# paroj/aruco

Measured on AMD Instinct MI355X. Metric: frames/sec at 1920×1080, higher is better.
Workload: dtype u8; 1 GPU; 1920x1080 synthetic stream, ~20 markers/frame, threshold+contour+decode+LINES, no pose (config 2); distinct_frames_per_gpu=1024, markers_rendered_per_frame=20, batches_in_flight=5, build=src=0ab799cac5660a2f flags=[], gpu_max_hw_queues=4, parallelism=frames sharded 1 stream/GPU

## Files before the change

### aruco_amd/csrc/decode_device.h

```cpp
#pragma once
#include "internal.h"

namespace ah {

__device__ inline bool solve8(double* A, double* b) {
    const int n = 8;
    for (int c = 0; c < n; c++) {
        int piv = c;
        double best = fabs(A[c * n + c]);
        for (int r = c + 1; r < n; r++) {
            double v = fabs(A[r * n + c]);
            if (v > best) best = v, piv = r;
        }
        if (best == 0) return false;
        if (piv != c) {
            for (int k = 0; k < n; k++) {
                double t = A[c * n + k];
                A[c * n + k] = A[piv * n + k];
                A[piv * n + k] = t;
            }
            double t = b[c];
            b[c] = b[piv];
            b[piv] = t;
        }
        double inv = 1.0 / A[c * n + c];
        for (int r = c + 1; r < n; r++) {
            double f = A[r * n + c] * inv;
            if (f == 0) continue;
            for (int k = c; k < n; k++) A[r * n + k] -= f * A[c * n + k];
            b[r] -= f * b[c];
        }
    }
    for (int r = n - 1; r >= 0; r--) {
        double s = b[r];
        for (int k = r + 1; k < n; k++) s -= A[r * n + k] * b[k];
        b[r] = s / A[r * n + r];
    }
    return true;
}

__device__ inline void perspective_transform_solve(const float* src, const float* dst, double* A, double* b, bool float_products = false) {
    for (int i = 0; i < 64; i++) A[i] = 0;
    for (int i = 0; i < 4; i++) {
        const float sx = src[2 * i], sy = src[2 * i + 1], dx = dst[2 * i], dy = dst[2 * i + 1];
        double* r0 = A + i * 8;
        double* r1 = A + (i + 4) * 8;
        r0[0] = r1[3] = sx;
        r0[1] = r1[4] = sy;
        r0[2] = r1[5] = 1;
        if (float_products) {
            r0[6] = -sx * dx;
            r0[7] = -sy * dx;
            r1[6] = -sx * dy;
            r1[7] = -sy * dy;
        } else {
            r0[6] = -(double)sx * dx;
            r0[7] = -(double)sy * dx;
            r1[6] = -(double)sx * dy;
            r1[7] = -(double)sy * dy;
        }
        b[i] = dx;
        b[i + 4] = dy;
    }
    if (!solve8(A, b))
        for (int i = 0; i < 8; i++) b[i] = 0;
}

constexpr int HOMOGRAPHY_GROUP = 16;
template <int G>
struct LaneMatT {
    double* base;
    int lane;
    __device__ __forceinline__ double& operator[](int k) const { return base[k * G + (lane & (G - 1))]; }
};
using LaneMat = LaneMatT<HOMOGRAPHY_GROUP>;
template <int G>
constexpr int homography_lds_doubles() { return 64 * G + 8 * G; }
constexpr int HOMOGRAPHY_LDS_DOUBLES = homography_lds_doubles<HOMOGRAPHY_GROUP>();

template <typename Mat>
__device__ __forceinline__ void homography_lane(const int16_t* qx, const int16_t* qy, int ws, const Mat& A, const Mat& b, double* iM) {
    const double d = (double)(float)(ws - 1);
    const double dxs[4] = {0, d, d, 0}, dys[4] = {0, 0, d, d};
    for (int i = 0; i < 64; i++) A[i] = 0;
    for (int i = 0; i < 4; i++) {
        const double sx = (double)(float)qx[i], sy = (double)(float)qy[i], dx = dxs[i], dy = dys[i];
        const int r0 = i * 8, r1 = (i + 4) * 8;
        A[r0 + 0] = sx, A[r1 + 3] = sx;
        A[r0 + 1] = sy, A[r1 + 4] = sy;
        A[r0 + 2] = 1, A[r1 + 5] = 1;
        A[r0 + 6] = -sx * dx;
        A[r0 + 7] = -sy * dx;
        A[r1 + 6] = -sx * dy;
        A[r1 + 7] = -sy * dy;
        b[i] = dx;
        b[i + 4] = dy;
    }
    bool ok = true;
    for (int c = 0; c < 8 && ok; c++) {
        int piv = c;
        double best = fabs(A[c * 8 + c]);
        for (int r = c + 1; r < 8; r++) {
            double v = fabs(A[r * 8 + c]);
            if (v > best) best = v, piv = r;
        }
        if (best == 0) {
            ok = false;
            break;
        }
        if (piv != c) {
            for (int k = 0; k < 8; k++) {
                double t = A[c * 8 + k];
                A[c * 8 + k] = A[piv * 8 + k];
                A[piv * 8 + k] = t;
            }
            double t = b[c];
            b[c] = b[piv];
            b[piv] = t;
        }
        const double inv = 1.0 / A[c * 8 + c];
        for (int r = c + 1; r < 8; r++) {
            const double f = A[r * 8 + c] * inv;
            if (f == 0) continue;
            for (int k = c; k < 8; k++) A[r * 8 + k] -= f * A[c * 8 + k];
            b[r] -= f * b[c];
        }
    }
    double m[9];
    if (ok) {
        for (int r = 7; r >= 0; r--) {
            double sacc = b[r];
            for (int k = r + 1; k < 8; k++) sacc -= A[r * 8 + k] * b[k];
            b[r] = sacc / A[r * 8 + r];
        }
        for (int i = 0; i < 8; i++) m[i] = b[i];
    } else {
        for (int i = 0; i < 8; i++) m[i] = 0;
    }
    m[8] = 1.0;
    double det = m[0] * (m[4] * m[8] - m[5] * m[7]) - m[1] * (m[3] * m[8] - m[5] * m[6]) + m[2] * (m[3] * m[7] - m[4] * m[6]);
    det = det != 0 ? 1. / det : 0;
    iM[0] = (m[4] * m[8] - m[5] * m[7]) * det;
    iM[1] = (m[2] * m[7] - m[1] * m[8]) * det;
    iM[2] = (m[1] * m[5] - m[2] * m[4]) * det;
    iM[3] = (m[5] * m[6] - m[3] * m[8]) * det;
    iM[4] = (m[0] * m[8] - m[2] * m[6]) * det;
    iM[5] = (m[2] * m[3] - m[0] * m[5]) * det;
    iM[6] = (m[3] * m[7] - m[4] * m[6]) * det;
    iM[7] = (m[1] * m[6] - m[0] * m[7]) * det;
    iM[8] = (m[0] * m[4] - m[1] * m[3]) * det;
}

__device__ __forceinline__ int hamm_rows(const uint32_t v[5]) {
    const uint32_t words[4] = {0x01, 0x1D, 0x12, 0x0E};
    int dist = 0;
#pragma unroll
    for (int y = 0; y < 5; y++) {
        int best = 100000;
#pragma unroll
        for (int p = 0; p < 4; p++) best = min(best, __popc(v[y] ^ words[p]));
        dist += best;
    }
    return dist;
}

__device__ __forceinline__ void fiducial_decode_word(unsigned long long m, int* id_out, int* nrot_out) {
    int id = -1, nrot = 0;
    unsigned long long border = 0x7Full | (0x7Full << 42);
#pragma unroll
    for (int y = 1; y < 6; y++) border |= (1ull << (7 * y)) | (1ull << (7 * y + 6));
    if ((m & border) == 0) {
        uint32_t cur[5], best[5];
#pragma unroll
        for (int y = 0; y < 5; y++) cur[y] = (uint32_t)(m >> (7 * (y + 1) + 1)) & 31u, best[y] = cur[y];
        int min_dist = hamm_rows(cur);
#pragma unroll
        for (int r = 1; r < 4; r++) {
            uint32_t nxt[5];
#pragma unroll
            for (int i = 0; i < 5; i++) {
                nxt[i] = 0;
#pragma unroll
                for (int j = 0; j < 5; j++) nxt[i] |= ((cur[4 - j] >> i) & 1u) << j;
            }
#pragma unroll
            for (int i = 0; i < 5; i++) cur[i] = nxt[i];
            const int dd = hamm_rows(cur);
            if (dd < min_dist) {
                min_dist = dd, nrot = r;
#pragma unroll
                for (int i = 0; i < 5; i++) best[i] = cur[i];
            }
        }
        if (min_dist == 0) {
            id = 0;
#pragma unroll
            for (int y = 0; y < 5; y++) id |= (int)((((best[y] >> 1) & 1u) << 1) | ((best[y] >> 3) & 1u)) << (2 * (4 - y));
        }
    }
    *id_out = id, *nrot_out = nrot;
}

constexpr int CELLS_PITCH = 8;
constexpr int cell_vote_rank(int sw) { return (sw * sw) / 2 + 1; }

__device__ __forceinline__ void cells_decode_wave(const uint8_t* patch, int ws, int thr, int lane, int* id_out, int* nrot_out) {
    const int sw = ws / 7;
    const int half = cell_vote_rank(sw) - 1;
    bool white = false;
    if (lane < 49) {
        const int cy = lane / 7, cx = lane - cy * 7;
        int cnt = 0;
        if (sw == 8 && (((size_t)patch | (size_t)ws) & 7) == 0) {
#pragma unroll
            for (int y = 0; y < 8; y++) {
                const uint2 w = *(const uint2*)(patch + (cy * 8 + y) * ws + cx * 8);
#pragma unroll
                for (int b = 0; b < 4; b++) cnt += (int)((w.x >> (8 * b)) & 0xFFu) > thr, cnt += (int)((w.y >> (8 * b)) & 0xFFu) > thr;
            }
        } else {
            for (int y = 0; y < sw; y++)
                for (int x = 0; x < sw; x++) cnt += patch[(cy * sw + y) * ws + cx * sw + x] > thr;
        }
        white = cnt > half;
    }
    const unsigned long long m = __ballot(white);
    int id = -1, nrot = 0;
    if (lane == 0) fiducial_decode_word(m, &id, &nrot);
    *id_out = id, *nrot_out = nrot;
}

}
```

### aruco_amd/csrc/k_contours.hip

```cpp
#include <algorithm>

#include "bits_tiles.h"
#include "internal.h"
#include "decode_device.h"

namespace ah {

__device__ __forceinline__ int first_dir(uint32_t m, int s_end) {
    int s = s_end;
    do {
        s = (s - 1) & 7;
        if ((m >> s) & 1) break;
    } while (s != s_end);
    return s == s_end ? -1 : s;
}

__device__ __forceinline__ bool run_rule_tiles(const uint64_t* __restrict__ tiles, int tnx, int x, int y, int hole) {
    int avail, avail_up;
    const uint64_t mid = tb_row64(tiles, tnx, x, y, &avail), up = tb_row64(tiles, tnx, x, y - 1, &avail_up);
    if (!hole) {
        int L = (~mid) ? __builtin_ctzll(~mid) : 64;
        L = min(L, avail);
        const int hi = min(L, avail - 1);
        const uint64_t m = hi >= 2 ? ((hi >= 63 ? ~0ull : ((1ull << (hi + 1)) - 1ull)) & ~3ull) : 0ull;
        return (up & m) == 0;
    }
    int L = mid ? __builtin_ctzll(mid) : 64;
    L = min(L, avail);
    const int hi = min(L - 1, avail - 1);
    const uint64_t m = hi >= 1 ? ((hi >= 63 ? ~0ull : ((1ull << (hi + 1)) - 1ull)) & ~1ull) : 0ull;
    return (~up & m) == 0;
}

struct CandArgs {
    const uint64_t* tiles;
    int tnx, tny;
    int width, height;
    uint32_t* trig_cnt;
    uint2* raw;
    uint32_t* raw_cnt;
    uint32_t* counters;
    uint32_t cap_raw;
    int grid_mask;
    uint32_t* hash;
    uint32_t hash_size;
};

constexpr int CAND_THREADS = 256;
constexpr int CAND_STAGE = 512;

__global__ __launch_bounds__(CAND_THREADS) void candidates_kernel(CandArgs a) {
    throughput_bound_priority();
    __shared__ uint2 s_keep[CAND_STAGE];
    __shared__ uint32_t s_n, s_base;
    const int plane = blockIdx.y;
    const uint64_t* __restrict__ tiles = a.tiles + (size_t)plane * a.tnx * a.tny;
    const int ntx = a.tnx - 1, nty = a.tny - 1;
    const int ntiles = ntx * nty;
    const uint64_t COL0 = 0x0101010101010101ull, COL7 = 0x8080808080808080ull;
    for (uint32_t i = blockIdx.x * CAND_THREADS + threadIdx.x; i < a.hash_size; i += gridDim.x * CAND_THREADS) a.hash[(size_t)plane * a.hash_size + i] = 0xFFFFFFFFu;
    uint2* const out = a.raw + (size_t)plane * a.cap_raw;
    uint32_t* const out_cnt = a.raw_cnt + plane * TRIG_CNT_STRIDE;

    auto stage = [&](uint2 rec) {
        const uint32_t ls = atomicAdd(&s_n, 1u);
        if (ls < CAND_STAGE) {
            s_keep[ls] = rec;
        } else {
            const uint32_t slot = atomicAdd(out_cnt, 1u);
            if (slot < a.cap_raw)
                out[slot] = rec;
            else
                flag_overflow(a.counters, a.trig_cnt, plane, ST_TRIG_OVERFLOW);
        }
    };

    for (int i0 = blockIdx.x * CAND_THREADS; i0 < ntiles; i0 += gridDim.x * CAND_THREADS) {
        if (threadIdx.x == 0) s_n = 0;
        __syncthreads();
        const int i = i0 + threadIdx.x;
        if (i < ntiles) {
            const int ty = i / ntx, tx = i - ty * ntx;
            const uint64_t* t = tiles + (size_t)ty * a.tnx + tx;
            const uint64_t T = t[0];
            const uint64_t L = tx > 0 ? t[-1] : 0ull;
            const uint64_t U = ty > 0 ? t[-a.tnx] : 0ull, UL = (ty > 0 && tx > 0) ? t[-a.tnx - 1] : 0ull, UR = ty > 0 ? t[-a.tnx + 1] : 0ull;
            const uint64_t Rt = t[1];
            if (T | L | U) {
                const uint64_t Wn = ((T << 1) & ~COL0) | ((L >> 7) & COL0);
                const uint64_t N = (T << 8) | (U >> 56), NLt = (L << 8) | (UL >> 56), NRt = (Rt << 8) | (UR >> 56);
                const uint64_t NW = ((N << 1) & ~COL0) | ((NLt >> 7) & COL0);
                const uint64_t NE = ((N >> 1) & ~COL7) | ((NRt << 7) & COL7);
                const int jmax = a.width - 2 - 8 * tx, imax = a.height - 2 - 8 * ty;
                const uint64_t colm = (jmax >= 7 ? 0xFFull : ((1ull << (jmax + 1)) - 1ull)) * COL0;
                const uint64_t rowm = imax >= 7 ? ~0ull : ((1ull << (8 * (imax + 1))) - 1ull);
                const uint64_t outer = T & ~(Wn | NW | N | NE);
                const uint64_t hole = ~T & Wn & N & colm & rowm;
                const uint32_t base = ((uint32_t)(8 * ty) << 16) | (uint32_t)(8 * tx);
                uint64_t rsel = 0, csel = 0;
#pragma unroll
                for (int q = 0; q < 8; q++) {
                    if (((8 * ty + q) & a.grid_mask) == 0) rsel |= 0xFFull << (8 * q);
                    if (((8 * tx + q) & a.grid_mask) == 0) csel |= COL0 << q;
                }
                const uint64_t crW = T & ~Wn & (rsel | outer);
                const uint64_t crE = ~T & Wn & (rsel | hole);
                const uint64_t crN = T & ~N & csel;
                const uint64_t crS = N & ~T & csel;
                for (int kind = 0; kind < 4; kind++) {
                    uint64_t m = kind == 0 ? crW : kind == 1 ? crE : kind == 2 ? crN : crS;
                    while (m) {
                        const int b = __builtin_ctzll(m);
                        m &= m - 1;
                        const uint32_t z = base + ((uint32_t)(b >> 3) << 16) + (uint32_t)(b & 7);
                        uint32_t pos, code, cand = 0;
                        if (kind == 0) pos = z, code = 2u, cand = (uint32_t)(outer >> b) & 1u;
                        else if (kind == 1) pos = z - 1u, code = 0u, cand = (uint32_t)(hole >> b) & 1u;
                        else if (kind == 2) pos = z, code = 1u;
                        else pos = z - 65536u, code = 3u;
                        stage(make_uint2(cand, (pos << 2) | code));
                    }
                }
            }
        }
        __syncthreads();
        if (threadIdx.x == 0 && s_n) s_base = atomicAdd(out_cnt, min(s_n, (uint32_t)CAND_STAGE));
        __syncthreads();
        const uint32_t n = min(s_n, (uint32_t)CAND_STAGE);
        for (uint32_t j = threadIdx.x; j < n; j += CAND_THREADS) {
            const uint32_t slot = s_base + j;
            if (slot < a.cap_raw)
                out[slot] = s_keep[j];
            else
                flag_overflow(a.counters, a.trig_cnt, plane, ST_TRIG_OVERFLOW);
        }
        __syncthreads();
    }
}

constexpr int CQ_CAP = 192;
constexpr int CS_CAP = 256;

struct SparseArgs {
    const uint64_t* tiles;
    const uint64_t* tile_bits;
    int tnx, tny, nstrips;
    int width, height;
    uint2* trig;
    uint32_t* trig_cnt;
    uint32_t* counters;
    uint32_t cap_trig;
    int drop_single;
};

__global__ __launch_bounds__(64) void candidates_sparse_kernel(SparseArgs a) {
    throughput_bound_priority();
    __shared__ uint32_t s_q[CQ_CAP];
    __shared__ uint2 s_keep[2][CS_CAP];
    __shared__ uint32_t s_n[2];
    const int plane = blockIdx.y, lane = threadIdx.x;
    const uint64_t* __restrict__ tiles = a.tiles + (size_t)plane * a.tnx * a.tny;
    const uint64_t* __restrict__ bits = a.tile_bits + (size_t)plane * a.tny * (2 * a.nstrips);
    const int ntx = a.tnx - 1, nty = a.tny - 1;
    const uint32_t half = a.cap_trig / 2;
    uint2* const out = a.trig + (size_t)plane * a.cap_trig;
    uint32_t* const out_cnt = a.trig_cnt + plane * TRIG_CNT_STRIDE;
    const uint64_t COL0 = 0x0101010101010101ull, COL7 = 0x8080808080808080ull;
    if (lane < 2) s_n[lane] = 0;
    __syncthreads();

    auto flush = [&]() {
        __syncthreads();
        for (int kind = 0; kind < 2; kind++) {
            const uint32_t n = min(s_n[kind], (uint32_t)CS_CAP);
            if (n == 0) continue;
            uint32_t base = 0;
            if (lane == 0) base = atomicAdd(&out_cnt[kind], n);
            base = (uint32_t)__builtin_amdgcn_readfirstlane((int)base);
            for (uint32_t j = lane; j < n; j += WAVE) {
                if (base + j < half)
                    out[(size_t)kind * half + base + j] = s_keep[kind][j];
                else
                    flag_overflow(a.counters, a.trig_cnt, plane, ST_TRIG_OVERFLOW);
            }
        }
        __syncthreads();
        if (lane < 2) s_n[lane] = 0;
        __syncthreads();
    };
    auto stage = [&](int kind, uint2 rec) {
        const uint32_t ls = atomicAdd(&s_n[kind], 1u);
        if (ls < CS_CAP) {
            s_keep[kind][ls] = rec;
        } else {
            const uint32_t slot = atomicAdd(&out_cnt[kind], 1u);
            if (slot < half)
                out[(size_t)kind * half + slot] = rec;
            else
                flag_overflow(a.counters, a.trig_cnt, plane, ST_TRIG_OVERFLOW);
        }
    };
    struct TileSet {
        uint64_t T, L, U, UL, UR, Rt;
        int tx, ty;
    };
    auto fetch = [&](bool live, uint32_t id) -> TileSet {
        TileSet q;
        q.ty = (int)(id >> 16), q.tx = (int)(id & 0xFFFFu);
        q.T = q.L = q.U = q.UL = q.UR = q.Rt = 0ull;
        if (live) {
            const uint64_t* t = tiles + (size_t)q.ty * a.tnx + q.tx;
            q.T = t[0];
            q.L = q.tx > 0 ? t[-1] : 0ull;
            q.U = q.ty > 0 ? t[-a.tnx] : 0ull, q.UL = (q.ty > 0 && q.tx > 0) ? t[-a.tnx - 1] : 0ull, q.UR = q.ty > 0 ? t[-a.tnx + 1] : 0ull;
            q.Rt = t[1];
        }
        return q;
    };
    auto evaluate = [&](bool live, const TileSet& q) {
        if (live) {
            const int ty = q.ty, tx = q.tx;
            const uint64_t T = q.T, L = q.L, U = q.U, UL = q.UL, UR = q.UR, Rt = q.Rt;
            const uint64_t Wn = ((T << 1) & ~COL0) | ((L >> 7) & COL0);
            const uint64_t N = (T << 8) | (U >> 56), NLt = (L << 8) | (UL >> 56), NRt = (Rt << 8) | (UR >> 56);
            const uint64_t NW = ((N << 1) & ~COL0) | ((NLt >> 7) & COL0);
            const uint64_t NE = ((N >> 1) & ~COL7) | ((NRt << 7) & COL7);
            const int jmax = a.width - 2 - 8 * tx, imax = a.height - 2 - 8 * ty;
            const uint64_t colm = (jmax >= 7 ? 0xFFull : (jmax < 0 ? 0ull : ((1ull << (jmax + 1)) - 1ull))) * COL0;
            const uint64_t rowm = imax >= 7 ? ~0ull : (imax < 0 ? 0ull : ((1ull << (8 * (imax + 1))) - 1ull));
            uint64_t outer = T & ~(Wn | NW | N | NE);
            const uint64_t hole = ~T & Wn & N & colm & rowm;
            if (a.drop_single) {
                const uint64_t E = ((T >> 1) & ~COL7) | ((Rt << 7) & COL7);
                const uint64_t lower = (T >> 8) | (Wn >> 8) | (E >> 8);
                outer &= ~(~(E | lower) & 0x00FFFFFFFFFFFFFFull);
            }
            const uint32_t base = ((uint32_t)(8 * ty) << 16) | (uint32_t)(8 * tx);
            uint64_t m = outer | hole;
            while (m) {
                const int b = __builtin_ctzll(m);
                m &= m - 1;
                const int qr = b >> 3, j = b & 7;
                const uint32_t kind = (uint32_t)(hole >> b) & 1u;
                const uint32_t mid = ((((uint32_t)(T >> (8 * qr)) & 0xFFu) | (((uint32_t)(Rt >> (8 * qr)) & 0xFFu) << 8)) >> j);
                const uint32_t up = ((((uint32_t)(N >> (8 * qr)) & 0xFFu) | (((uint32_t)(NRt >> (8 * qr)) & 0xFFu) << 8)) >> j);
                const int avail = 16 - j;
                const uint32_t pos = base + ((uint32_t)qr << 16) + (uint32_t)j;
                const uint32_t runbits = (kind ? mid : ~mid) | (1u << avail);
                const int Lr = __builtin_ctz(runbits);
                const int hi = kind ? min(Lr - 1, avail - 1) : min(Lr, avail - 1);
                const uint32_t span = ((2u << hi) - 1u) & (kind ? ~1u : ~3u);
                if (((kind ? ~up : up) & span) != 0) continue;
                if (Lr < avail || run_rule_tiles(tiles, a.tnx, (int)(pos & 0xFFFFu), (int)(pos >> 16), (int)kind)) stage((int)kind, make_uint2(kind, pos));
            }
        }
        __syncthreads();
        if (max(s_n[0], s_n[1]) > CS_CAP - 64) flush();
    };

    const int nw = 2 * a.nstrips;
    auto row_words = [&](int ty) -> uint64_t {
        const int which = lane / nw, idx = lane - which * nw, row = ty - which;
        return (ty < nty && which < 2 && row >= 0) ? bits[(size_t)row * nw + idx] : 0ull;
    };
    auto word_of = [&](uint64_t v, int l) -> uint64_t {
        return (uint64_t)(uint32_t)__builtin_amdgcn_readlane((int)(uint32_t)v, l) | ((uint64_t)(uint32_t)__builtin_amdgcn_readlane((int)(uint32_t)(v >> 32), l) << 32);
    };
    uint32_t qn = 0;
    uint64_t nextw = row_words(blockIdx.x);
    for (int ty = blockIdx.x; ty < nty; ty += gridDim.x) {
        const uint64_t curw = nextw;
        nextw = row_words(ty + gridDim.x);
        for (int st = 0; st < a.nstrips; st++) {
            const uint64_t A = word_of(curw, 2 * st), Bm = word_of(curw, 2 * st + 1);
            const uint64_t UA = word_of(curw, nw + 2 * st), UB = word_of(curw, nw + 2 * st + 1);
            const uint64_t carry = st > 0 ? (word_of(curw, 2 * st - 1) >> 63) : 0ull;
            const uint64_t needA = A | (Bm << 1) | carry | UA, needB = Bm | A | UB;
#pragma unroll
            for (int odd = 0; odd < 2; odd++) {
                const uint64_t need = odd ? needB : needA;
                const int tx = 128 * st + 2 * lane + odd;
                const bool act = ((need >> lane) & 1ull) && tx < ntx;
                const unsigned long long bal = __ballot(act);
                if (bal) {
                    if (act) s_q[qn + (uint32_t)__popcll(bal & ((1ull << lane) - 1ull))] = ((uint32_t)ty << 16) | (uint32_t)tx;
                    qn += (uint32_t)__popcll(bal);
                    __syncthreads();
                    if (qn >= 128) {
                        qn -= 128;
                        const TileSet q0 = fetch(true, s_q[qn + 64 + lane]), q1 = fetch(true, s_q[qn + lane]);
                        evaluate(true, q0);
                        evaluate(true, q1);
                    }
                }
            }
        }
    }
    {
        const bool l0 = qn >= 64 ? true : (uint32_t)lane < qn;
        const bool l1 = qn >= 64 && (uint32_t)lane < qn - 64;
        const TileSet q0 = fetch(l0, l0 ? s_q[lane] : 0u), q1 = fetch(l1, l1 ? s_q[64 + lane] : 0u);
        if (qn > 0) evaluate(l0, q0);
        if (qn > 64) evaluate(l1, q1);
    }
    flush();
}
// ... 680 lines not shown
        }
        --top;
        const int sl_start = s_stack[top][0], sl_end = s_stack[top][1];
        __syncthreads();
        const short2 ep = P[sl_end], sp = P[sl_start];
        int len = sl_end - sl_start;
        if (len <= 0) len += count;
        bool small;
        int split = 0;
        if (len > 1) {
            const int dx = ep.x - sp.x, dy = ep.y - sp.y;
            const uint32_t w = ((uint32_t)(-dy) & 0xFFFFu) | ((uint32_t)dx << 16);
            uint32_t bd, bq, maxd_u, qmax;
            scan_cyclic<true>(PW, count, sl_start + 1 == count ? 0 : sl_start + 1, len - 1, lane, PW[sl_start], w, bd, bq);
            wave_argmax_first(bd, bq, &maxd_u, &qmax);
            double maxd = (double)maxd_u;
            int q = qmax == 0xFFFFFFFFu ? 0 : (int)qmax;
            split = sl_start + 1 + q;
            if (split >= count) split -= count;
            small = maxd * maxd <= eps * ((double)dx * (double)dx + (double)dy * (double)dy);
        } else {
            small = true;
        }
        if (small) {
            if (lane == 0) s_out[outn] = sp;
            outn++;
        } else {
            if (lane == 0) {
                s_stack[top][0] = split, s_stack[top][1] = sl_end;
                s_stack[top + 1][0] = sl_start, s_stack[top + 1][1] = split;
            }
            top += 2;
        }
        __syncthreads();
    }
    if (reject || outn < 4) return;
    if (lane == 0) polygon_to_quad(a, cd, ci, s_out, outn, eps);
}

#ifndef DUAL_MAX_N
#define DUAL_MAX_N 512
#endif
constexpr int DUAL_MAX = DUAL_MAX_N;
__device__ __forceinline__ void border_pair_to_quads(const QuadArgs& a, const ContourDesc& cd, const uint32_t ci, const bool valid, short2* Pbase, int (*s_stack)[16][2],
                                                     short2 (*s_out)[12], uint32_t* rows) {
    const int lane = threadIdx.x, h = lane >> 5, hl = lane & 31;
    const bool upper = h != 0;
    short2* P = Pbase + h * DUAL_MAX;
    uint32_t* P32 = (uint32_t*)P;
    const int count = valid ? cd.n : 1;
    if (a.from_pool) {
        if (valid)
            for (int i = hl; i < count; i += 32) P[i] = a.pool[cd.pool_off + i];
    } else {
        const uint64_t* tiles = a.tiles + (size_t)cd.plane * a.tnx * a.tny;
        const int ncp = (count + CK - 1) / CK;
        const uint32_t* ckp = cd.ck_off == 0xFFFFFFFFu ? (const uint32_t*)(a.pool + cd.pool_off) - ncp : a.walk_scratch + cd.ck_off;
        const uint32_t* rb = rows + lane - 64;
        for (int k = hl; k < (DUAL_MAX + CK - 1) / CK; k += 32) {
            if (!(valid && k < ncp)) continue;
            const uint32_t c = ckp[k];
            const uint32_t pos = (c & 0x3FFFu) | (((c >> 14) & 0x3FFFu) << 16);
            const int n0 = k * CK, n1 = min(n0 + CK, count);
            int bx, by;
            if (k + 1 < ncp) {
                const uint32_t cn = ckp[k + 1];
                bx = (int)(cn & 0x3FFFu), by = (int)((cn >> 14) & 0x3FFFu);
            } else {
                bx = cd.x0, by = cd.y0;
            }
            const int ax = (int)(pos & 0xFFFFu), ay = (int)(pos >> 16), L = n1 - n0;
            const int ex = (L - abs(bx - ax)) >> 1, ey = (L - abs(by - ay)) >> 1;
            const int tx0 = min(max((min(ax, bx) - ex - 1) >> 3, 0), a.tnx - 4), ty0 = min(max((min(ay, by) - ey - 1) >> 3, 0), a.tny - 4);
            TileBlock blk;
            tb_load_at<64>(tiles, a.tnx, tx0, ty0, rows, lane, blk);
            const uint32_t base1 = tb_base1(blk);
            uint32_t lp = pos - base1, s1c = tb_s1c((int)(c >> 28));
#pragma unroll
            for (int j = 0; j < CK; j++) {
                if (n0 + j < n1) {
                    P32[n0 + j] = lp + base1;
                    tb_step<64>(rb, lp, s1c);
                }
            }
        }
    }
    __syncthreads();
    if (!a.from_pool && valid)
        for (int i = hl; i < count; i += 32) a.pool[cd.pool_off + i] = P[i];

    double eps = (double)count * 0.05;
    eps *= eps;
    int pos = 0, rs_start = 0;
    bool le_eps = false;
    const uint32_t* PW = (const uint32_t*)P;
    for (int it = 0; it < 3; it++) {
        pos = (pos + rs_start) % count;
        uint32_t bd, bk, maxd, kmax;
        scan_cyclic<false, 32>(PW, count, pos + 1 == count ? 0 : pos + 1, count - 1, hl, PW[pos], 0u, bd, bk);
        half_argmax_first(bd, bk, upper, &maxd, &kmax);
        if (maxd > 0) rs_start = (int)kmax + 1;
        le_eps = (double)maxd <= eps;
    }
    int top = 0, outn = 0;
    bool reject = !valid;
    if (!le_eps) {
        const int sl_start = pos % count;
        const int sl_end = (rs_start + sl_start) % count;
        if (hl == 0) {
            s_stack[h][0][0] = sl_end, s_stack[h][0][1] = sl_start;
            s_stack[h][1][0] = sl_start, s_stack[h][1][1] = sl_end;
        }
        top = 2;
    } else {
        if (hl == 0) s_out[h][0] = P[pos];
        outn = 1;
    }
    __syncthreads();
    for (;;) {
        bool act = !reject && top > 0;
        if (act && outn + top > 8) reject = true, act = false;
        if (!__any(act)) break;
        int sl_start = 0, sl_end = 0, len = 0;
        short2 ep = make_short2(0, 0), sp = make_short2(0, 0);
        uint32_t bd = 0, bq = 0xFFFFFFFFu;
        int dx = 0, dy = 0;
        if (act) {
            --top;
            sl_start = s_stack[h][top][0], sl_end = s_stack[h][top][1];
            ep = P[sl_end], sp = P[sl_start];
            len = sl_end - sl_start;
            if (len <= 0) len += count;
            if (len > 1) {
                dx = ep.x - sp.x, dy = ep.y - sp.y;
                const uint32_t w = ((uint32_t)(-dy) & 0xFFFFu) | ((uint32_t)dx << 16);
                scan_cyclic<true, 32>(PW, count, sl_start + 1 == count ? 0 : sl_start + 1, len - 1, hl, PW[sl_start], w, bd, bq);
            }
        }
        __syncthreads();
        uint32_t maxd_u, qmax;
        half_argmax_first(bd, bq, upper, &maxd_u, &qmax);
        if (act) {
            bool small = true;
            int split = 0;
            if (len > 1) {
                const double maxd = (double)maxd_u;
                const int q = qmax == 0xFFFFFFFFu ? 0 : (int)qmax;
                split = sl_start + 1 + q;
                if (split >= count) split -= count;
                small = maxd * maxd <= eps * ((double)dx * (double)dx + (double)dy * (double)dy);
            }
            if (small) {
                if (hl == 0) s_out[h][outn] = sp;
                outn++;
            } else {
                if (hl == 0) {
                    s_stack[h][top][0] = split, s_stack[h][top][1] = sl_end;
                    s_stack[h][top + 1][0] = sl_start, s_stack[h][top + 1][1] = split;
                }
                top += 2;
            }
        }
        __syncthreads();
    }
    if (hl == 0 && !reject && outn >= 4) polygon_to_quad(a, cd, ci, s_out[h], outn, eps);
}

__device__ __forceinline__ void quad_blocks(const QuadArgs& a, const int bid, short2* Plds, uint32_t* rows, int (*s_stack)[16][2], short2 (*s_out)[12], int& s_outn) {
    const int xcd = bid & 7, rest = bid >> 3;
    const int chunk = rest % a.qblocks, plane = (rest / a.qblocks) * 8 + xcd;
    if (plane >= a.nplanes) return;
    const uint32_t nall = min(a.trig_cnt[plane * TRIG_CNT_STRIDE + TC_CDESC], a.cap_cdesc);
    const uint32_t nsnap = min(a.trig_cnt[plane * TRIG_CNT_STRIDE + TC_SNAP], a.cap_cdesc);
    const uint32_t nlate = a.pass == 3 ? min(a.trig_cnt[plane * TRIG_CNT_STRIDE + TC_LATE], a.cap_cdesc - nall) : 0u;
    const uint32_t lo = a.pass == 2 ? nsnap : 0u, ncd = a.pass == 3 ? nlate : a.pass == 1 ? nsnap : nall;
    const bool upper = threadIdx.x >= 32;
    ContourDesc pend;
    uint32_t pend_ci = 0;
    bool has_pend = false;
    for (uint32_t cslot = lo + (uint32_t)chunk; cslot < ncd; cslot += (uint32_t)a.qblocks) {
        const uint32_t ci = (uint32_t)plane * a.cap_cdesc + (a.pass == 3 ? a.cap_cdesc - 1u - cslot : cslot);
        const ContourDesc cd = a.cdesc[ci];
        if (cd.n <= 0) continue;
        if (a.dual && cd.n <= DUAL_MAX) {
            if (!has_pend) {
                pend = cd, pend_ci = ci, has_pend = true;
                continue;
            }
            __syncthreads();
            border_pair_to_quads(a, upper ? cd : pend, upper ? ci : pend_ci, true, Plds, s_stack, s_out, rows);
            has_pend = false;
            continue;
        }
        __syncthreads();
        if (cd.n <= QP_LDS)
            border_to_quad<true>(a, cd, ci, Plds, s_stack[0], s_out[0], s_outn, rows);
        else
            border_to_quad<false>(a, cd, ci, a.pool + cd.pool_off, s_stack[0], s_out[0], s_outn, rows);
    }
    if (has_pend) {
        __syncthreads();
        border_to_quad<true>(a, pend, pend_ci, Plds, s_stack[0], s_out[0], s_outn, rows);
    }
}

__global__ __launch_bounds__(64) void contour_quad_kernel(QuadArgs a) {
    throughput_bound_priority();
    __shared__ __align__(16) short2 Plds[QP_LDS];
    __shared__ uint32_t rows[TB_ROWS * EMIT_LANES];
    __shared__ int s_stack[2][16][2];
    __shared__ short2 s_out[2][12];
    __shared__ int s_outn;
    static_assert(QP_LDS >= 2 * DUAL_MAX && EMIT_LANES == 64, "the two-borders-per-wave path uses the whole point buffer and a block per lane");
    quad_blocks(a, blockIdx.x, Plds, rows, s_stack, s_out, s_outn);
}

struct LateQuadArgs {
    WalkArgs w;
    QuadArgs q;
};
__global__ __launch_bounds__(64) void late_quad_kernel(LateQuadArgs a) {
    __shared__ __align__(16) short2 Plds[QP_LDS];
    __shared__ uint32_t rows[TB_ROWS * EMIT_LANES];
    __shared__ int s_stack[2][16][2];
    __shared__ short2 s_out[2][12];
    __shared__ int s_outn;
    static_assert(EMIT_LANES == 64, "the late walks use the quad role's blocks: one per lane");
    const int nwalk = 2 * a.w.gen_blocks;
    if ((int)blockIdx.x < nwalk) {
        latency_bound_priority();
        if ((int)blockIdx.x < a.w.gen_blocks)
            walk_generation<false, true>(a.w, blockIdx.x, rows);
        else
            walk_generation<true, true>(a.w, blockIdx.x - a.w.gen_blocks, rows);
        return;
    }
    throughput_bound_priority();
    quad_blocks(a.q, (int)blockIdx.x - nwalk, Plds, rows, s_stack, s_out, s_outn);
}

static int quad_blocks_per_plane(int nplanes) {
    constexpr int kBlocks = 12;
    return nplanes <= 2 ? 128 : nplanes <= 8 ? 48 : kBlocks;
}

static QuadArgs quad_args(const FrameGeom& g, int nframes, const DetectParams& p, const Buffers& b, int pass) {
    QuadArgs a;
    a.pass = pass;
    a.tiles = b.tiles, a.tnx = tiles_x(g.width), a.tny = tiles_y(g.height), a.from_pool = b.seg_mode, a.cdesc = b.cdesc, a.pool = b.pool, a.quads = b.quads, a.counters = b.counters;
    a.cap_cdesc = b.cap_cdesc, a.cap_quads = b.cap_quads, a.nthr = p.nthr, a.width = g.width, a.height = g.height;
    a.trig_cnt = b.trig_cnt, a.walk_scratch = b.walk_scratch;
    a.nplanes = nframes * p.nthr;
    a.dual = b.env.quad_dual && a.nplanes > 8;
    const int qb = quad_blocks_per_plane(a.nplanes);
    a.qblocks = pass == 2 ? std::max(1, qb / 2) : qb;
    return a;
}

void launch_contour_quads(hipStream_t s, const FrameGeom& g, int nframes, const DetectParams& p, const Buffers& b, int pass) {
    const QuadArgs a = quad_args(g, nframes, p, b, pass);
    const int planes8 = ((a.nplanes + 7) / 8) * 8;
    hipLaunchKernelGGL(contour_quad_kernel, dim3(planes8 * a.qblocks), dim3(64), 0, s, a);
}

void launch_late_quads(hipStream_t s, const FrameGeom& g, int nframes, const DetectParams& p, const Buffers& b) {
    LateQuadArgs a;
    a.w = walk_args(g, nframes * p.nthr, p, b);
    a.w.gen = GEN_FORK_AFTER + 1, a.w.gen_steps = p.max_contour;
    int before = a.w.leash;
    for (int gen = 1; gen <= GEN_FORK_AFTER; gen++) before += gen_steps_of(gen, p);
    a.w.gen_blocks = gen_blocks_of(a.w.nplanes, before);
    a.q = quad_args(g, nframes, p, b, 0);
    const int planes8 = ((a.q.nplanes + 7) / 8) * 8;
    hipLaunchKernelGGL(late_quad_kernel, dim3(2 * a.w.gen_blocks + planes8 * a.q.qblocks), dim3(64), 0, s, a);
    launch_contour_quads(s, g, nframes, p, b, 3);
}

struct FrameArgs {
    double* iM;
    int ws;
    const Quad* quads;
    Cand* cands;
    uint32_t* cand_list;
    uint32_t cap_flat;
    int32_t* ncands;
    uint32_t* counters;
    uint32_t* trig_cnt;
    int nthr;
    int cap_quads, cap_cands;
};

constexpr int MAXQ = 512;

__device__ __forceinline__ float quad_perimeter_i(const int16_t* x, const int16_t* y) {
    float sum = 0;
    for (int i = 0; i < 4; i++) {
        int j = (i + 1) & 3;
        double dx = (double)(x[i] - x[j]), dy = (double)(y[i] - y[j]);
        sum = (float)((double)sum + sqrt(dx * dx + dy * dy));
    }
    return sum;
}

template <int HG>
__global__ __launch_bounds__(64) void frame_candidates_kernel(FrameArgs a) {
    latency_bound_priority();
    constexpr int PHASE1_BYTES = MAXQ * (8 + 8 + 4 + 4 + 2 + 1 + 1);
    constexpr int BIG_DOUBLES = homography_lds_doubles<HG>() > (PHASE1_BYTES + 7) / 8 ? homography_lds_doubles<HG>() : (PHASE1_BYTES + 7) / 8;
    __shared__ double s_big[BIG_DOUBLES];
    int16_t(*sx)[4] = (int16_t(*)[4])s_big;
    int16_t(*sy)[4] = sx + MAXQ;
    int* s_cdesc = (int*)(sy + MAXQ);
    float* s_perim = (float*)(s_cdesc + MAXQ);
    int16_t* s_map = (int16_t*)(s_perim + MAXQ);
    uint8_t* s_swapped = (uint8_t*)(s_map + MAXQ);
    uint8_t* s_rem = s_swapped + MAXQ;
    __shared__ int s_n;
    __shared__ uint32_t s_base;
    const int frame = blockIdx.x, lane = threadIdx.x;
    const int nq = min((int)a.counters[CNT_FIXED + frame], min(a.cap_quads, MAXQ));
    const Quad* Q = a.quads + (size_t)frame * a.cap_quads;
    for (int i = lane; i < nq; i += WAVE) {
        const uint32_t key = Q[i].key;
        int rank = 0;
        for (int j = 0; j < nq; j++) rank += Q[j].key < key;
        Quad q = Q[i];
        int d1x = q.x[1] - q.x[0], d1y = q.y[1] - q.y[0], d2x = q.x[2] - q.x[0], d2y = q.y[2] - q.y[0];
        float o = ((float)d1x * (float)d2y) - ((float)d1y * (float)d2x);
        bool sw = o < 0.0f;
        if (sw) {
            int16_t tx = q.x[1], ty = q.y[1];
            q.x[1] = q.x[3], q.y[1] = q.y[3];
            q.x[3] = tx, q.y[3] = ty;
        }
        for (int k = 0; k < 4; k++) sx[rank][k] = q.x[k], sy[rank][k] = q.y[k];
        s_cdesc[rank] = q.cdesc;
        s_swapped[rank] = sw;
        s_rem[rank] = 0;
        s_perim[rank] = quad_perimeter_i(q.x, q.y);
    }
    __syncthreads();
    for (int i = 0; i < nq; i++) {
        for (int j = i + 1 + lane; j < nq; j += WAVE) {
            bool near = true;
            for (int c = 0; c < 4; c++) {
                int dx = sx[i][c] - sx[j][c], dy = sy[i][c] - sy[j][c];
                near = near && (dx * dx + dy * dy < 36);
            }
            if (near) {
                if (s_perim[i] > s_perim[j])
                    s_rem[j] = 1;
                else
                    s_rem[i] = 1;
            }
        }
    }
    __syncthreads();
    if (lane == 0) {
        int n = 0;
        Cand* C = a.cands + (size_t)frame * a.cap_cands;
        for (int i = 0; i < nq; i++) {
            if (s_rem[i]) continue;
            if (n >= a.cap_cands) {
                flag_overflow(a.counters, a.trig_cnt, frame * a.nthr, ST_CAND_OVERFLOW);
                break;
            }
            Cand c;
            for (int k = 0; k < 4; k++) {
                c.c[2 * k] = (float)sx[i][k], c.c[2 * k + 1] = (float)sy[i][k];
                c.qx[k] = sx[i][k], c.qy[k] = sy[i][k];
            }
            c.cdesc = s_cdesc[i], c.swapped = s_swapped[i], c.id = -1, c.nrot = 0;
            s_map[n] = (int16_t)i;
            C[n++] = c;
        }
        a.ncands[frame] = n;
        uint32_t base = 0;
        if (n > 0) {
            base = atomicAdd(&a.counters[CNT_NCAND], (uint32_t)n);
            for (int i = 0; i < n; i++) {
                if (base + i < a.cap_flat)
                    a.cand_list[base + i] = ((uint32_t)frame << 16) | (uint32_t)i;
                else
                    flag_overflow(a.counters, a.trig_cnt, frame * a.nthr, ST_CAND_OVERFLOW);
            }
        }
        s_n = n, s_base = base;
    }
    __syncthreads();
    const int n = s_n;
    const uint32_t base = s_base;
    constexpr int PER_LANE = MAXQ / WAVE;
    int16_t qx[PER_LANE][4], qy[PER_LANE][4];
#pragma unroll
    for (int r = 0; r < PER_LANE; r++) {
        const int k = r * WAVE + lane;
        if (k < n) {
            const int i = s_map[k];
            for (int c = 0; c < 4; c++) qx[r][c] = sx[i][c], qy[r][c] = sy[i][c];
        } else {
            for (int c = 0; c < 4; c++) qx[r][c] = 0, qy[r][c] = 0;
        }
    }
    __syncthreads();
    const LaneMatT<HG> A{s_big, lane}, b{s_big + 64 * HG, lane};
#pragma unroll
    for (int r = 0; r < PER_LANE; r++) {
        if (r * WAVE >= n) break;
        const int k = r * WAVE + lane;
        for (int g = 0; g < WAVE / HG; g++) {
            if (r * WAVE + g * HG >= n) break;
            if (lane / HG == g && k < n && base + (uint32_t)k < a.cap_flat)
                homography_lane(qx[r], qy[r], a.ws, A, b, a.iM + (size_t)(base + (uint32_t)k) * 9);
        }
    }
}

void launch_frame_candidates(hipStream_t s, const FrameGeom& g, int nframes, const DetectParams& p, const Buffers& b) {
    FrameArgs a;
    a.quads = b.quads, a.cands = b.cands, a.ncands = b.ncands, a.counters = b.counters, a.trig_cnt = b.trig_cnt, a.nthr = p.nthr;
    a.cand_list = b.cand_list, a.cap_flat = b.cap_flat;
    a.cap_quads = b.cap_quads, a.cap_cands = b.cap_cands;
    a.iM = b.iM, a.ws = p.warp_size;
    if (nframes <= 2)
        hipLaunchKernelGGL(frame_candidates_kernel<64>, dim3(nframes), dim3(64), 0, s, a);
    else
        hipLaunchKernelGGL(frame_candidates_kernel<HOMOGRAPHY_GROUP>, dim3(nframes), dim3(64), 0, s, a);
}

}
```

Baseline: 442,100 frames/s.

## Parallelize candidate dedup, compaction and homography solve across wave lanes

Reworks frame_candidates_kernel so that each lane computes a quad's sort rank and near-duplicate removal in one pass, replacing the separate O(n^2) rank loop and the serial pairwise marking. Candidate compaction and cand_list writes now use ballot/popcount across the wave instead of a single lane, with 16-byte vector stores. The 8x8 homography solve is redistributed so 8 lanes each hold one matrix row in registers and exchange rows via shuffles, removing the LDS-backed per-lane matrix and the group-serialized loop. This trades LDS traffic and serial lane-0 work for more cross-lane shuffles and a register-tracked pivot permutation.

```diff
diff --git a/aruco_amd/csrc/cand_compact.h b/aruco_amd/csrc/cand_compact.h
--- /dev/null
+++ b/aruco_amd/csrc/cand_compact.h
@@ -0,0 +1,20 @@
+#pragma once
+#include <stdint.h>
+
+#if defined(__HIPCC__)
+#define CAND_COMPACT_HD __host__ __device__
+#else
+#define CAND_COMPACT_HD
+#endif
+
+namespace ah {
+
+CAND_COMPACT_HD inline int compact_index(unsigned long long kept, int lane, int base) {
+    return base + __builtin_popcountll(kept & ((1ull << lane) - 1ull));
+}
+
+CAND_COMPACT_HD inline int kept_candidates(int survivors, int cap_cands) { return survivors < cap_cands ? survivors : cap_cands; }
+
+CAND_COMPACT_HD inline bool flat_entry_fits(uint32_t base, int k, uint32_t cap_flat) { return base + (uint32_t)k < cap_flat; }
+
+}
diff --git a/aruco_amd/csrc/decode_device.h b/aruco_amd/csrc/decode_device.h
--- a/aruco_amd/csrc/decode_device.h
+++ b/aruco_amd/csrc/decode_device.h
@@ -66,80 +66,64 @@
         for (int i = 0; i < 8; i++) b[i] = 0;
 }
 
-constexpr int HOMOGRAPHY_GROUP = 16;
-template <int G>
-struct LaneMatT {
-    double* base;
-    int lane;
-    __device__ __forceinline__ double& operator[](int k) const { return base[k * G + (lane & (G - 1))]; }
-};
-using LaneMat = LaneMatT<HOMOGRAPHY_GROUP>;
-template <int G>
-constexpr int homography_lds_doubles() { return 64 * G + 8 * G; }
-constexpr int HOMOGRAPHY_LDS_DOUBLES = homography_lds_doubles<HOMOGRAPHY_GROUP>();
-
-template <typename Mat>
-__device__ __forceinline__ void homography_lane(const int16_t* qx, const int16_t* qy, int ws, const Mat& A, const Mat& b, double* iM) {
+__device__ __forceinline__ double homography_rows8(double sx, double sy, int ws, int lane, double* iM8) {
+    const int r = lane & 7, g0 = lane & ~7, i = r & 3;
     const double d = (double)(float)(ws - 1);
-    const double dxs[4] = {0, d, d, 0}, dys[4] = {0, 0, d, d};
-    for (int i = 0; i < 64; i++) A[i] = 0;
-    for (int i = 0; i < 4; i++) {
-        const double sx = (double)(float)qx[i], sy = (double)(float)qy[i], dx = dxs[i], dy = dys[i];
-        const int r0 = i * 8, r1 = (i + 4) * 8;
-        A[r0 + 0] = sx, A[r1 + 3] = sx;
-        A[r0 + 1] = sy, A[r1 + 4] = sy;
-        A[r0 + 2] = 1, A[r1 + 5] = 1;
-        A[r0 + 6] = -sx * dx;
-        A[r0 + 7] = -sy * dx;
-        A[r1 + 6] = -sx * dy;
-        A[r1 + 7] = -sy * dy;
-        b[i] = dx;
-        b[i + 4] = dy;
-    }
+    const double dx = (i == 1 || i == 2) ? d : 0, dy = i >= 2 ? d : 0;
+    const double t = r < 4 ? dx : dy;
+    double a[8], bb = t;
+#pragma unroll
+    for (int k = 0; k < 8; k++) a[k] = 0;
+    if (r < 4)
+        a[0] = sx, a[1] = sy, a[2] = 1;
+    else
+        a[3] = sx, a[4] = sy, a[5] = 1;
+    a[6] = -sx * t;
+    a[7] = -sy * t;
+    uint32_t perm = 0x76543210u;
+    int myl = r;
     bool ok = true;
-    for (int c = 0; c < 8 && ok; c++) {
+#pragma unroll
+    for (int c = 0; c < 8; c++) {
         int piv = c;
-        double best = fabs(A[c * 8 + c]);
-        for (int r = c + 1; r < 8; r++) {
-            double v = fabs(A[r * 8 + c]);
-            if (v > best) best = v, piv = r;
-        }
-        if (best == 0) {
-            ok = false;
-            break;
-        }
-        if (piv != c) {
-            for (int k = 0; k < 8; k++) {
-                double t = A[c * 8 + k];
-                A[c * 8 + k] = A[piv * 8 + k];
-                A[piv * 8 + k] = t;
-            }
-            double t = b[c];
-            b[c] = b[piv];
-            b[piv] = t;
-        }
-        const double inv = 1.0 / A[c * 8 + c];
-        for (int r = c + 1; r < 8; r++) {
-            const double f = A[r * 8 + c] * inv;
-            if (f == 0) continue;
-            for (int k = c; k < 8; k++) A[r * 8 + k] -= f * A[c * 8 + k];
-            b[r] -= f * b[c];
+        double best = fabs(__shfl(a[c], g0 + (int)((perm >> (4 * c)) & 7u)));
+#pragma unroll
+        for (int l = c + 1; l < 8; l++) {
+            const double v = fabs(__shfl(a[c], g0 + (int)((perm >> (4 * l)) & 7u)));
+            if (v > best) best = v, piv = l;
+        }
+        if (best == 0) ok = false;
+        const uint32_t lc = (perm >> (4 * c)) & 7u, lp = (perm >> (4 * piv)) & 7u;
+        perm = (perm & ~(0xFu << (4 * c)) & ~(0xFu << (4 * piv))) | (lp << (4 * c)) | (lc << (4 * piv));
+        myl = myl == c ? piv : myl == piv ? c : myl;
+        double p[8];
+#pragma unroll
+        for (int k = c; k < 8; k++) p[k] = __shfl(a[k], g0 + (int)lp);
+        const double pb = __shfl(bb, g0 + (int)lp);
+        const double inv = 1.0 / p[c];
+        const double f = a[c] * inv;
+        if (myl > c && !(f == 0)) {
+#pragma unroll
+            for (int k = c + 1; k < 8; k++) a[k] -= f * p[k];
+            bb -= f * pb;
         }
     }
     double m[9];
-    if (ok) {
-        for (int r = 7; r >= 0; r--) {
-            double sacc = b[r];
-            for (int k = r + 1; k < 8; k++) sacc -= A[r * 8 + k] * b[k];
-            b[r] = sacc / A[r * 8 + r];
-        }
-        for (int i = 0; i < 8; i++) m[i] = b[i];
-    } else {
-        for (int i = 0; i < 8; i++) m[i] = 0;
+#pragma unroll
+    for (int l = 7; l >= 0; l--) {
+        double sacc = bb;
+#pragma unroll
+        for (int k = l + 1; k < 8; k++) sacc -= a[k] * m[k];
+        m[l] = __shfl(sacc / a[l], g0 + (int)((perm >> (4 * l)) & 7u));
+    }
+    if (!ok) {
+#pragma unroll
+        for (int k = 0; k < 8; k++) m[k] = 0;
     }
     m[8] = 1.0;
     double det = m[0] * (m[4] * m[8] - m[5] * m[7]) - m[1] * (m[3] * m[8] - m[5] * m[6]) + m[2] * (m[3] * m[7] - m[4] * m[6]);
     det = det != 0 ? 1. / det : 0;
+    double iM[9];
     iM[0] = (m[4] * m[8] - m[5] * m[7]) * det;
     iM[1] = (m[2] * m[7] - m[1] * m[8]) * det;
     iM[2] = (m[1] * m[5] - m[2] * m[4]) * det;
@@ -149,6 +133,11 @@
     iM[6] = (m[3] * m[7] - m[4] * m[6]) * det;
     iM[7] = (m[1] * m[6] - m[0] * m[7]) * det;
     iM[8] = (m[0] * m[4] - m[1] * m[3]) * det;
+    *iM8 = iM[8];
+    double out = iM[0];
+#pragma unroll
+    for (int k = 1; k < 8; k++) out = r == k ? iM[k] : out;
+    return out;
 }
 
 __device__ __forceinline__ int hamm_rows(const uint32_t v[5]) {
diff --git a/aruco_amd/csrc/k_contours.hip b/aruco_amd/csrc/k_contours.hip
--- a/aruco_amd/csrc/k_contours.hip
+++ b/aruco_amd/csrc/k_contours.hip
@@ -2,6 +2,7 @@
 
 #include "bits_tiles.h"
 #include "internal.h"
+#include "cand_compact.h"
 #include "decode_device.h"
 
 namespace ah {
@@ -1288,28 +1289,24 @@
     return sum;
 }
 
-template <int HG>
+struct __align__(16) QuadXY {
+    int16_t x[4], y[4];
+};
+constexpr int FC_LDS_BYTES = MAXQ * (16 + 4 + 4 + 4 + 2 + 1 + 1);
 __global__ __launch_bounds__(64) void frame_candidates_kernel(FrameArgs a) {
     latency_bound_priority();
-    constexpr int PHASE1_BYTES = MAXQ * (8 + 8 + 4 + 4 + 2 + 1 + 1);
-    constexpr int BIG_DOUBLES = homography_lds_doubles<HG>() > (PHASE1_BYTES + 7) / 8 ? homography_lds_doubles<HG>() : (PHASE1_BYTES + 7) / 8;
-    __shared__ double s_big[BIG_DOUBLES];
-    int16_t(*sx)[4] = (int16_t(*)[4])s_big;
-    int16_t(*sy)[4] = sx + MAXQ;
-    int* s_cdesc = (int*)(sy + MAXQ);
-    float* s_perim = (float*)(s_cdesc + MAXQ);
-    int16_t* s_map = (int16_t*)(s_perim + MAXQ);
-    uint8_t* s_swapped = (uint8_t*)(s_map + MAXQ);
-    uint8_t* s_rem = s_swapped + MAXQ;
-    __shared__ int s_n;
-    __shared__ uint32_t s_base;
+    __shared__ QuadXY s_q[MAXQ];
+    __shared__ uint32_t s_key[MAXQ];
+    __shared__ float s_perim[MAXQ];
+    __shared__ int s_cdesc[MAXQ];
+    __shared__ int16_t s_map[MAXQ];
+    __shared__ uint8_t s_swapped[MAXQ];
+    __shared__ uint8_t s_rem[MAXQ];
+    static_assert(sizeof(s_q) + sizeof(s_key) + sizeof(s_perim) + sizeof(s_cdesc) + sizeof(s_map) + sizeof(s_swapped) + sizeof(s_rem) == FC_LDS_BYTES, "LDS of frame_candidates_kernel");
     const int frame = blockIdx.x, lane = threadIdx.x;
     const int nq = min((int)a.counters[CNT_FIXED + frame], min(a.cap_quads, MAXQ));
     const Quad* Q = a.quads + (size_t)frame * a.cap_quads;
     for (int i = lane; i < nq; i += WAVE) {
-        const uint32_t key = Q[i].key;
-        int rank = 0;
-        for (int j = 0; j < nq; j++) rank += Q[j].key < key;
         Quad q = Q[i];
         int d1x = q.x[1] - q.x[0], d1y = q.y[1] - q.y[0], d2x = q.x[2] - q.x[0], d2y = q.y[2] - q.y[0];
         float o = ((float)d1x * (float)d2y) - ((float)d1y * (float)d2x);
@@ -1319,85 +1316,95 @@
             q.x[1] = q.x[3], q.y[1] = q.y[3];
             q.x[3] = tx, q.y[3] = ty;
         }
-        for (int k = 0; k < 4; k++) sx[rank][k] = q.x[k], sy[rank][k] = q.y[k];
-        s_cdesc[rank] = q.cdesc;
-        s_swapped[rank] = sw;
-        s_rem[rank] = 0;
-        s_perim[rank] = quad_perimeter_i(q.x, q.y);
+        QuadXY v;
+        for (int k = 0; k < 4; k++) v.x[k] = q.x[k], v.y[k] = q.y[k];
+        s_q[i] = v;
+        s_key[i] = q.key;
+        s_cdesc[i] = q.cdesc;
+        s_swapped[i] = sw;
+        s_perim[i] = quad_perimeter_i(q.x, q.y);
     }
     __syncthreads();
-    for (int i = 0; i < nq; i++) {
-        for (int j = i + 1 + lane; j < nq; j += WAVE) {
-            bool near = true;
+    for (int j = lane; j < nq; j += WAVE) {
+        const QuadXY mine = s_q[j];
+        const uint32_t key = s_key[j];
+        const float perim = s_perim[j];
+        int rank = 0;
+        bool rem = false;
+        for (int i = 0; i < nq; i++) {
+            const QuadXY o = s_q[i];
+            const uint32_t okey = s_key[i];
+            rank += okey < key;
+            bool near = i != j;
             for (int c = 0; c < 4; c++) {
-                int dx = sx[i][c] - sx[j][c], dy = sy[i][c] - sy[j][c];
+                int dx = o.x[c] - mine.x[c], dy = o.y[c] - mine.y[c];
                 near = near && (dx * dx + dy * dy < 36);
             }
             if (near) {
-                if (s_perim[i] > s_perim[j])
-                    s_rem[j] = 1;
-                else
-                    s_rem[i] = 1;
-            }
-        }
+                const float operim = s_perim[i];
+                rem = rem || (okey < key ? operim > perim : !(perim > operim));
+            }
+        }
+        s_map[rank] = (int16_t)j;
+        s_rem[j] = rem;
     }
     __syncthreads();
+    Cand* C = a.cands + (size_t)frame * a.cap_cands;
+    int survivors = 0;
+    for (int r0 = 0; r0 < nq; r0 += WAVE) {
+        const int rank = r0 + lane;
+        int j = 0;
+        bool keep = false;
+        if (rank < nq) j = s_map[rank] & (MAXQ - 1), keep = !s_rem[j];
+        const unsigned long long kept = __ballot(keep);
+        const int k = compact_index(kept, lane, survivors);
+        if (keep && k < a.cap_cands) {
+            const QuadXY v = s_q[j];
+            Cand c;
+            for (int e = 0; e < 4; e++) {
+                c.c[2 * e] = (float)v.x[e], c.c[2 * e + 1] = (float)v.y[e];
+                c.qx[e] = v.x[e], c.qy[e] = v.y[e];
+            }
+            c.cdesc = s_cdesc[j], c.swapped = s_swapped[j], c.id = -1, c.nrot = 0;
+            static_assert(sizeof(Cand) == 64, "a Cand is four 16-byte stores");
+            uint4 v4[4];
+            __builtin_memcpy(v4, &c, sizeof(c));
+            uint4* dst = (uint4*)(C + k);
+            for (int e = 0; e < 4; e++) dst[e] = v4[e];
+            s_map[k] = (int16_t)j;
+        }
+        survivors += __popcll(kept);
+    }
+    const int n = kept_candidates(survivors, a.cap_cands);
+    uint32_t base = 0;
     if (lane == 0) {
-        int n = 0;
-        Cand* C = a.cands + (size_t)frame * a.cap_cands;
-        for (int i = 0; i < nq; i++) {
-            if (s_rem[i]) continue;
-            if (n >= a.cap_cands) {
-                flag_overflow(a.counters, a.trig_cnt, frame * a.nthr, ST_CAND_OVERFLOW);
-                break;
-            }
-            Cand c;
-            for (int k = 0; k < 4; k++) {
-                c.c[2 * k] = (float)sx[i][k], c.c[2 * k + 1] = (float)sy[i][k];
-                c.qx[k] = sx[i][k], c.qy[k] = sy[i][k];
-            }
-            c.cdesc = s_cdesc[i], c.swapped = s_swapped[i], c.id = -1, c.nrot = 0;
-            s_map[n] = (int16_t)i;
-            C[n++] = c;
-        }
+        if (survivors > a.cap_cands) flag_overflow(a.counters, a.trig_cnt, frame * a.nthr, ST_CAND_OVERFLOW);
         a.ncands[frame] = n;
-        uint32_t base = 0;
-        if (n > 0) {
-            base = atomicAdd(&a.counters[CNT_NCAND], (uint32_t)n);
-            for (int i = 0; i < n; i++) {
-                if (base + i < a.cap_flat)
-                    a.cand_list[base + i] = ((uint32_t)frame << 16) | (uint32_t)i;
-                else
-                    flag_overflow(a.counters, a.trig_cnt, frame * a.nthr, ST_CAND_OVERFLOW);
-            }
-        }
-        s_n = n, s_base = base;
-    }
+        if (n > 0) base = atomicAdd(&a.counters[CNT_NCAND], (uint32_t)n);
+    }
+    base = __shfl(base, 0);
+    bool past_flat = false;
+    for (int k = lane; k < n; k += WAVE) {
+        if (flat_entry_fits(base, k, a.cap_flat))
+            a.cand_list[base + k] = ((uint32_t)frame << 16) | (uint32_t)k;
+        else
+            past_flat = true;
+    }
+    if (__ballot(past_flat) != 0 && lane == 0) flag_overflow(a.counters, a.trig_cnt, frame * a.nthr, ST_CAND_OVERFLOW);
     __syncthreads();
-    const int n = s_n;
-    const uint32_t base = s_base;
-    constexpr int PER_LANE = MAXQ / WAVE;
-    int16_t qx[PER_LANE][4], qy[PER_LANE][4];
-#pragma unroll
-    for (int r = 0; r < PER_LANE; r++) {
-        const int k = r * WAVE + lane;
+    for (int k0 = 0; k0 < n; k0 += WAVE / 8) {
+        const int k = k0 + (lane >> 3);
+        double sx = 0, sy = 0;
         if (k < n) {
-            const int i = s_map[k];
-            for (int c = 0; c < 4; c++) qx[r][c] = sx[i][c], qy[r][c] = sy[i][c];
-        } else {
-            for (int c = 0; c < 4; c++) qx[r][c] = 0, qy[r][c] = 0;
-        }
-    }
-    __syncthreads();
-    const LaneMatT<HG> A{s_big, lane}, b{s_big + 64 * HG, lane};
-#pragma unroll
-    for (int r = 0; r < PER_LANE; r++) {
-        if (r * WAVE >= n) break;
-        const int k = r * WAVE + lane;
-        for (int g = 0; g < WAVE / HG; g++) {
-            if (r * WAVE + g * HG >= n) break;
-            if (lane / HG == g && k < n && base + (uint32_t)k < a.cap_flat)
-                homography_lane(qx[r], qy[r], a.ws, A, b, a.iM + (size_t)(base + (uint32_t)k) * 9);
+            const int j = s_map[k];
+            sx = (double)(float)s_q[j].x[lane & 3], sy = (double)(float)s_q[j].y[lane & 3];
+        }
+        double m8;
+        const double m = homography_rows8(sx, sy, a.ws, lane, &m8);
+        if (k < n && flat_entry_fits(base, k, a.cap_flat)) {
+            double* iM = a.iM + (size_t)(base + (uint32_t)k) * 9;
+            iM[lane & 7] = m;
+            if ((lane & 7) == 0) iM[8] = m8;
         }
     }
 }
@@ -1408,10 +1415,7 @@
     a.cand_list = b.cand_list, a.cap_flat = b.cap_flat;
     a.cap_quads = b.cap_quads, a.cap_cands = b.cap_cands;
     a.iM = b.iM, a.ws = p.warp_size;
-    if (nframes <= 2)
-        hipLaunchKernelGGL(frame_candidates_kernel<64>, dim3(nframes), dim3(64), 0, s, a);
-    else
-        hipLaunchKernelGGL(frame_candidates_kernel<HOMOGRAPHY_GROUP>, dim3(nframes), dim3(64), 0, s, a);
-}
-
-}
+    hipLaunchKernelGGL(frame_candidates_kernel, dim3(nframes), dim3(64), 0, s, a);
+}
+
+}
```

After: 441,200 frames/s. No clear change (-0.2%).
